# artonson/autoinst

Hardware: AMD Instinct MI355X
Metric: chunks/sec (200k-pt TARL+Spatial NCuts chunk: affinity build + recursive normalized cut) (higher is better)
Workload: dtype f64; 1 GPU; configs[1]: single 200k-point surface chunk, TARL(96-d)+Spatial affinities, alpha=1 theta=0.5 T=0.03; per GPU per step 2 batched calls of 12 chunks (one pool of iterating segments each) taken from a queue by 2 host threads; 1 builder thread(s) build the next batches' affinity graphs meanwhile; n_points=200000, nnz=7311156, threads_per_gpu=2, builder_threads_per_gpu=1, chunks_per_batch=12, parallelism=chunk-dp1

## Files before the change

autoinst_amd/csrc/ai_affinity.hip:

```cpp
#include <cstring>

#include <rocprim/device/device_radix_sort.hpp>

#include "ai_common.h"

namespace {

struct Grid {
  double minx, miny, minz, inv_cell;
  int nx, ny, nz;
};

__device__ __forceinline__ uint32_t part1by2(uint32_t x) {
  x &= 0x3ffu;
  x = (x ^ (x << 16)) & 0xff0000ffu;
  x = (x ^ (x << 8)) & 0x0300f00fu;
  x = (x ^ (x << 4)) & 0x030c30c3u;
  x = (x ^ (x << 2)) & 0x09249249u;
  return x;
}

__device__ __forceinline__ void cell_of(const Grid& g, double x, double y, double z, int& cx, int& cy, int& cz) {
  cx = (int)floor((x - g.minx) * g.inv_cell);
  cy = (int)floor((y - g.miny) * g.inv_cell);
// ... 682 lines not shown
  AI_TRY(idx.alloc(n));
  hipLaunchKernelGGL(k_cell_keys, dim3(gb), dim3(AI_BLOCK), 0, st, d_xyz, n, g, key.p, idx.p);
  AI_KERNEL_CHECK();

  ai_csr* A = new ai_csr();
  A->n = n;
  A->nnz = 0;
  A->rowptr = nullptr;
  A->col = nullptr;
  A->val = nullptr;
  A->orig = nullptr;
  A->device = ctx->device;
  ai_register_graph(ctx, A);
  auto fail = [&](int s) {
    ai_csr_free(ctx, A);
    return s;
  };
#define AI_TRYF(expr)                \
  do {                               \
    int _s = (expr);                 \
    if (_s != AI_OK) return fail(_s); \
  } while (0)
#define AI_HIPF(expr)                                                                     \
  do {                                                                                    \
    hipError_t _e = (expr);                                                               \
    if (_e != hipSuccess) {                                                               \
      ai_set_error("%s:%d: %s -> %s", __FILE__, __LINE__, #expr, hipGetErrorString(_e)); \
      return fail((_e == hipErrorOutOfMemory) ? AI_ERR_OOM : AI_ERR_HIP);                \
    }                                                                                     \
  } while (0)

  AI_HIPF(ctx->graphs.alloc((void**)&A->orig, (size_t)n * sizeof(int32_t)));
  AI_HIPF(ctx->graphs.alloc((void**)&A->rowptr, (size_t)(n + 1) * sizeof(int32_t)));
  {
    size_t tmp_bytes = 0;
    AI_HIPF(rocprim::radix_sort_pairs(nullptr, tmp_bytes, key.p, key2.p, idx.p, A->orig, (size_t)n, 0, 30, st));
    DevBuf<uint8_t> tmp;
    AI_TRYF(tmp.alloc(tmp_bytes));
    AI_HIPF(rocprim::radix_sort_pairs(tmp.p, tmp_bytes, key.p, key2.p, idx.p, A->orig, (size_t)n, 0, 30, st));
    if (!ai_current_arena()) AI_HIPF(hipStreamSynchronize(st));
  }
  AI_TRYF(X.alloc(n));
  AI_TRYF(Y.alloc(n));
  AI_TRYF(Z.alloc(n));
  AI_TRYF(cellid.alloc(n));
  AI_TRYF(cstart.alloc(ncell));
  AI_TRYF(cend.alloc(ncell));
  AI_TRYF(cnt.alloc(n + 1));
  AI_TRYF(scantmp.alloc(ai_scan_tmp_elems(n)));
  hipLaunchKernelGGL(k_gather_sorted, dim3(gb), dim3(AI_BLOCK), 0, st, d_xyz, A->orig, n, g, X.p, Y.p, Z.p, cellid.p);
  AI_HIPF(hipGetLastError());
  AI_HIPF(hipMemsetAsync(cstart.p, 0xff, (size_t)ncell * sizeof(int32_t), st));
  AI_HIPF(hipMemsetAsync(cend.p, 0, (size_t)ncell * sizeof(int32_t), st));
  hipLaunchKernelGGL(k_cell_ranges, dim3(gb), dim3(AI_BLOCK), 0, st, cellid.p, n, cstart.p, cend.p);
  AI_HIPF(hipGetLastError());
  const unsigned gnb = (unsigned)((n * AI_NB_LANES + AI_BLOCK - 1) / AI_BLOCK);
  constexpr int AI_NB_STASH = 128;
  DevBuf<int32_t> stash_col;
  DevBuf<double> stash_dist;
  AI_TRYF(stash_col.alloc((size_t)n * AI_NB_STASH));
  AI_TRYF(stash_dist.alloc((size_t)n * AI_NB_STASH));
  hipLaunchKernelGGL(k_neighbours<false>, dim3(gnb), dim3(AI_BLOCK), 0, st, X.p, Y.p, Z.p, cellid.p, cstart.p, cend.p, n, g,
                     radius, cnt.p, (const int32_t*)nullptr, (int32_t*)nullptr, (double*)nullptr, stash_col.p, stash_dist.p, AI_NB_STASH,
                     (const int32_t*)nullptr);
  AI_HIPF(hipGetLastError());
  DevBuf<unsigned long long> total;
// ... 120 lines not shown
```

autoinst_amd/csrc/ai_api.hip:

```cpp
#include <stdarg.h>
#include <string.h>

#include <algorithm>
#include <stdlib.h>
#include <hip/hip_ext.h>
#include "ai_common.h"

static thread_local char g_err[1024] = "";

void ai_set_error(const char* fmt, ...) {
  va_list ap;
  va_start(ap, fmt);
  vsnprintf(g_err, sizeof(g_err), fmt, ap);
  va_end(ap);
}

extern "C" const char* ai_last_error(void) { return g_err; }
extern "C" int ai_abi_version(void) { return AI_ABI_VERSION; }
extern "C" int64_t ai_abi_sizeof(int which) {
  return which == 0 ? (int64_t)sizeof(ai_ncut_opts) : which == 1 ? (int64_t)sizeof(ai_ncut_stats) : -1;
}

static thread_local ai_arena* g_arena = nullptr;
ai_arena* ai_current_arena() { return g_arena; }
// ... 255 lines not shown
  out[3] = (int64_t)ctx->graphs.cached_bytes;
  return AI_OK;
}

extern "C" int ai_ctx_destroy(ai_ctx* ctx) {
  if (!ctx) return AI_OK;
  ctx->helper.stop();
  (void)hipSetDevice(ctx->device);
  if (ctx->stream) (void)hipStreamSynchronize(ctx->stream);
  for (int i = 0; i < 8; ++i)
    if (ctx->ev[i]) (void)hipEventDestroy(ctx->ev[i]);
  if (ctx->side) (void)hipStreamSynchronize(ctx->side);
  for (int i = 0; i < AI_CHECK_DEPTH; ++i) {
    if (ctx->chk_ev[i]) (void)hipEventDestroy(ctx->chk_ev[i]);
    if (ctx->chk_ev1[i]) (void)hipEventDestroy(ctx->chk_ev1[i]);
  }
  if (ctx->side) (void)hipStreamDestroy(ctx->side);
  if (ctx->wave) {
    (void)hipStreamSynchronize(ctx->wave);
    (void)hipStreamDestroy(ctx->wave);
  }
  for (int i = 0; i < AI_FLOW_EVENTS; ++i)
    if (ctx->fev[i]) (void)hipEventDestroy(ctx->fev[i]);
  if (ctx->fpin) (void)hipHostFree(ctx->fpin);
  if (ctx->pinned) (void)hipHostFree(ctx->pinned);
  if (ctx->stage) (void)hipHostFree(ctx->stage);
  {
    std::lock_guard<std::mutex> lock(ctx->graphs_mu);
    for (ai_csr* g : ctx->live_graphs) {
      g->rowptr = nullptr;
      g->col = nullptr;
      g->val = nullptr;
      g->orig = nullptr;
      g->owner = nullptr;
    }
    ctx->live_graphs.clear();
  }
  ctx->arena.release_all();
  ctx->graphs.release_all();
  if (ctx->stream) (void)hipStreamDestroy(ctx->stream);
  delete ctx;
  return AI_OK;
}

extern "C" int ai_csr_free(ai_ctx* ctx, ai_csr* csr) {
  (void)ctx;
  if (!csr) return AI_OK;
  if (ai_ctx* o = csr->owner) {
    (void)hipSetDevice(o->device);
    {
      std::lock_guard<std::mutex> lock(o->graphs_mu);
      for (size_t i = 0; i < o->live_graphs.size(); ++i)
        if (o->live_graphs[i] == csr) {
          o->live_graphs.erase(o->live_graphs.begin() + i);
          break;
        }
    }
    o->graphs.release(csr->rowptr);
    o->graphs.release(csr->col);
    o->graphs.release(csr->val);
    o->graphs.release(csr->orig);
  }
  delete csr;
  return AI_OK;
}

extern "C" int ai_csr_dims(const ai_csr* csr, int64_t* n, int64_t* nnz) {
  if (!csr) {
    ai_set_error("ai_csr_dims: csr is null");
    return AI_ERR_BAD_ARG;
  }
  if (n) *n = csr->n;
  if (nnz) *nnz = csr->nnz;
  return AI_OK;
}

extern "C" int ai_csr_from_host(ai_ctx* ctx, int64_t n, const int64_t* indptr, const int32_t* indices, const double* data,
                                ai_csr** out) {
  if (!ctx || !indptr || !out || n <= 0) {
    ai_set_error("ai_csr_from_host: bad argument");
    return AI_ERR_BAD_ARG;
  }
  const int64_t nnz = indptr[n];
  if (indptr[0] != 0 || nnz < 0 || nnz >= ((int64_t)1 << 31) || n >= ((int64_t)1 << 30) || (nnz > 0 && (!indices || !data))) {
    ai_set_error("ai_csr_from_host: indptr[0] = %lld, nnz = %lld out of range", (long long)indptr[0], (long long)nnz);
    return AI_ERR_BAD_ARG;
  }
  std::vector<int32_t> rp((size_t)n + 1);
  for (int64_t i = 0; i <= n; ++i) {
    if (i > 0 && indptr[i] < indptr[i - 1]) {
      ai_set_error("ai_csr_from_host: indptr decreases at row %lld", (long long)i);
      return AI_ERR_BAD_ARG;
    }
    rp[(size_t)i] = (int32_t)indptr[i];
// ... 116 lines not shown
```

autoinst_amd/csrc/ai_common.h:

```cpp
#pragma once
#include <hip/hip_runtime.h>
#include <stdint.h>
#include <stdio.h>
#include <condition_variable>
#include <functional>
#include <mutex>
#include <atomic>
#include <thread>
#include <string>
#include <vector>

#include "../../include/autoinst_hip.h"

void ai_set_error(const char* fmt, ...);

#define AI_HIP(expr)                                                                      \
  do {                                                                                    \
    hipError_t _e = (expr);                                                               \
    if (_e != hipSuccess) {                                                               \
      ai_set_error("%s:%d: %s -> %s", __FILE__, __LINE__, #expr, hipGetErrorString(_e)); \
      return (_e == hipErrorOutOfMemory) ? AI_ERR_OOM : AI_ERR_HIP;                      \
    }                                                                                     \
  } while (0)

// ... 86 lines not shown
  hipEvent_t ev[8];
  int num_cu;
  int32_t* pinned;
  hipEvent_t chk_ev[AI_CHECK_DEPTH];
  hipEvent_t chk_ev1[AI_CHECK_DEPTH];
  hipStream_t side;
  hipStream_t wave = nullptr;
  char* fpin = nullptr;
  hipEvent_t fev[AI_FLOW_EVENTS] = {};
  ai_arena arena;
  ai_graph_cache graphs;
  char* stage;
  std::mutex graphs_mu;
  std::vector<ai_csr*> live_graphs;
  ai_helper helper;
};
void ai_register_graph(ai_ctx* ctx, ai_csr* g);
#define AI_CHECK_GRAPH(g, who)                                          \
  do {                                                                  \
    if ((g) && !(g)->rowptr) {                                          \
      ai_set_error("%s: the graph's context was destroyed", (who));     \
      return AI_ERR_BAD_ARG;                                            \
    }                                                                   \
  } while (0)

struct ai_csr {
  int64_t n;
  int64_t nnz;
  int32_t* rowptr;
  int32_t* col;
  double* val;
  int32_t* orig;
  int device;
  ai_ctx* owner = nullptr;
};

template <typename T>
struct DevBuf {
  T* p = nullptr;
  size_t count = 0;
  bool owned = false;
  DevBuf() {}
  DevBuf(const DevBuf&) = delete;
  DevBuf& operator=(const DevBuf&) = delete;
  ~DevBuf() { release(); }
  void release() {
    if (p && owned) (void)hipFree(p);
    p = nullptr;
    count = 0;
    owned = false;
  }
  int alloc(size_t n) {
    release();
    if (n == 0) n = 1;
    if (ai_arena* a = ai_current_arena()) {
      p = (T*)a->alloc(n * sizeof(T));
      if (!p) {
        ai_set_error("device workspace of %zu bytes could not be allocated", n * sizeof(T));
        return AI_ERR_OOM;
      }
      count = n;
      return AI_OK;
    }
    hipError_t e = hipMalloc((void**)&p, n * sizeof(T));
    if (e != hipSuccess) {
      p = nullptr;
// ... 114 lines not shown
```

autoinst_amd/csrc/ai_dense_sym.h:

```cpp
#pragma once
#include <algorithm>
#include <cmath>
#include <vector>

inline void cf_jacobi(std::vector<double> a, int B, std::vector<double>& evals, std::vector<double>& q) {
  q.assign((size_t)B * B, 0.0);
  for (int i = 0; i < B; ++i) q[(size_t)i * B + i] = 1.0;
  for (int sweep = 0; sweep < 60; ++sweep) {
    double off = 0.0, diag = 0.0;
    for (int i = 0; i < B; ++i) {
      diag += a[(size_t)i * B + i] * a[(size_t)i * B + i];
      for (int j = i + 1; j < B; ++j) off += a[(size_t)i * B + j] * a[(size_t)i * B + j];
    }
    if (off <= 1e-32 * std::max(diag, 1e-300)) break;
    for (int p = 0; p < B - 1; ++p)
      for (int r = p + 1; r < B; ++r) {
        const double apr = a[(size_t)p * B + r];
        if (fabs(apr) < 1e-300) continue;
        const double app = a[(size_t)p * B + p], arr = a[(size_t)r * B + r];
        const double tau = (arr - app) / (2.0 * apr);
        const double t = (tau >= 0.0 ? 1.0 : -1.0) / (fabs(tau) + sqrt(1.0 + tau * tau));
        const double c = 1.0 / sqrt(1.0 + t * t), s = t * c;
        for (int k = 0; k < B; ++k) {
          const double akp = a[(size_t)k * B + p], akr = a[(size_t)k * B + r];
          a[(size_t)k * B + p] = c * akp - s * akr;
          a[(size_t)k * B + r] = s * akp + c * akr;
        }
        for (int k = 0; k < B; ++k) {
          const double apk = a[(size_t)p * B + k], ark = a[(size_t)r * B + k];
          a[(size_t)p * B + k] = c * apk - s * ark;
          a[(size_t)r * B + k] = s * apk + c * ark;
        }
        for (int k = 0; k < B; ++k) {
          const double qkp = q[(size_t)k * B + p], qkr = q[(size_t)k * B + r];
          q[(size_t)k * B + p] = c * qkp - s * qkr;
          q[(size_t)k * B + r] = s * qkp + c * qkr;
// ... 156 lines not shown
```

autoinst_amd/csrc/ai_flow.inc:

```

struct RangeAlloc {
  std::map<int, int> fr;
  void init(int cap) {
    fr.clear();
    fr[0] = cap;
  }
  int alloc(int n) {
    for (auto it = fr.begin(); it != fr.end(); ++it)
      if (it->second >= n) {
        const int b = it->first, len = it->second;
        fr.erase(it);
        if (len > n) fr[b + n] = len - n;
        return b;
      }
    return -1;
  }
  void release(int b, int n) {
    auto it = fr.emplace(b, n).first;
    auto nx = std::next(it);
    if (nx != fr.end() && it->first + it->second == nx->first) {
      it->second += nx->second;
      fr.erase(nx);
    }
    if (it != fr.begin()) {
      auto pv = std::prev(it);
      if (pv->first + pv->second == it->first) {
        pv->second += it->second;
        fr.erase(it);
      }
    }
  }
};

struct FSeg {
  int g0 = 0, n = 0, chunk = 0, par = 0;
  int slot = -1;
  int t0 = 0, cap = 0;
  int f0 = -1, c0 = -1;
  int m = 0;
  int aux = 0;
  bool frozen = false;
  bool binary_child = false;
  int vdelta = 0;
  int warm_n = 0;
  int restarts = 0;
  double prev_true = 0.0;
};

static inline int fk_nf(int n) { return (n + AI_FINE_ROWS - 1) / AI_FINE_ROWS; }
static inline int fk_nc(int n) { return (n + AI_COARSE_ROWS - 1) / AI_COARSE_ROWS; }

class Flow {
 public:
  static constexpr int RING = 16;
  static constexpr size_t UPSLOT_BYTES = (size_t)256 << 10;
  static constexpr size_t PIN_UP = AI_FLOW_UPSLOTS * UPSLOT_BYTES;
  static constexpr size_t STATUS_BYTES = (size_t)64 << 10;
  static constexpr size_t PIN_STATUS = STATUS_BYTES;
  static constexpr size_t PIN_RES = (size_t)1 << 20;
  static constexpr size_t PIN_HIST = (size_t)16 << 20;
  static constexpr size_t PIN_COEF = (size_t)8 << 20;
  static constexpr size_t PIN_TOTAL = PIN_UP + PIN_STATUS + PIN_RES + PIN_HIST + PIN_COEF;
  static constexpr int TS_CAP = 1 << 16;
  static constexpr int AHEAD = 10;
  static constexpr int AHEAD_SMALL = 8;

  explicit Flow(ai_ctx* c) : ctx(c), sm(c->stream), ss(c->side) {}
  ai_ctx* ctx;
  hipStream_t sm, ss, sw = nullptr;
  ai_ncut_opts opt{1e-10, 4000, 16, 0, 0};
  bool clock_spmv = false;
  ai_ncut_stats stats{};
  int N = 0;
  int64_t E = 0;
  int nchunks = 0;
  const int64_t* off = nullptr;
  const int64_t* n_orig = nullptr;
  double T = 0.0;
  int SMAX = 0, WCAP = 0, FCAP = 0, CCAP = 0, FLIST = 0, CLIST = 0, mcap = 0;
  int W = 0;
  RangeAlloc sa;
  std::vector<int> chunk_sbase, chunk_live;
  std::deque<int> waiting;
  std::vector<FSeg> new_roots;
  int64_t window_rows = 0;
  FlowCsr G{};
  DevBuf<int2> rowse0, rowse1;
  DevBuf<int32_t> col1, orig1;
  DevBuf<double> w1;
  DevBuf<double> deg, sinv, sinv2, u1, wm, ev, Z;
  DevBuf<double> ev2, warmv;
  int warm = (getenv("AI_FLOW_WARM") && atoi(getenv("AI_FLOW_WARM")) == 0) ? 0 : 1;
  DevBuf<uint8_t> bin;
  DevBuf<int32_t> flag, fscan, map, newcnt, nscan, parent, rcnt, rc, ord, key, key_out, val, sorted_rows, final_order, scantmp;
  DevBuf<uint8_t> sorttmp;
  DevBuf<uint16_t> lidx;
  DevBuf<int32_t> ucol;
  DevBuf<TaskEnc> enc;
  DevBuf<int32_t> factive, cactive;
  DevBuf<double> pA;
  DevBuf<double2> pB0, pB1;
  DevBuf<int32_t> s_frozen, s_m, s_lastm, s_nextm;
  DevBuf<double> s_theta, s_resid, alpha_hist, b_hist, g_hist;
#ifdef AI_TRACE_HIST
  DevBuf<int4> sig_i, chk_i;
  DevBuf<double2> sig_d;
  DevBuf<double> chk_d;
#endif
  DevBuf<unsigned long long> work, tstamps, tblock;
  DevBuf<int32_t> dprog;
  DevBuf<int32_t> chk_ctr, chk_queue;
  DevBuf<double*> d_slabtab;
  DevBuf<FTask> d_ft[RING];
  DevBuf<CTask> d_ct[RING];
  DevBuf<PoolSeg> d_ps[RING];
  DevBuf<SegRec> d_poolrec;
  DevBuf<SegRec> wrecP, wrecC;
  DevBuf<Task> fineP, coarseP, fineC, coarseC;
  DevBuf<double> pvol, psweep, w_scale, w_thr, w_vol, coef_d;
  DevBuf<double2> presid;
  long long n_restarted = 0;
  const char* guard_log = getenv("AI_FLOW_GUARD_LOG");
  std::vector<double> hist_copy;
  std::vector<double> coef_copy;
  double max_true_resid = 0.0;
// ... 134 lines not shown
  int sync_slabtab() {
    if (slabtab_n == slabs.size()) return AI_OK;
    if (slabs.size() > 500) {
      ai_set_error("internal: more than 500 Lanczos slabs");
      return AI_ERR_INTERNAL;
    }
    double** tab = (double**)(pin_res() + PIN_RES / 2);
    for (size_t i = 0; i < slabs.size(); ++i) tab[i] = slabs[i];
    AI_HIP(hipMemcpyAsync(d_slabtab.p, tab, slabs.size() * sizeof(double*), hipMemcpyHostToDevice, sm));
    slabtab_n = slabs.size();
    return AI_OK;
  }

  static void make_recs(const std::vector<FSeg>& segs, std::vector<SegRec>& out, int& nf, int& nc) {
    out.resize(segs.size());
    nf = nc = 0;
    for (size_t i = 0; i < segs.size(); ++i) {
      const FSeg& s = segs[i];
      SegRec r;
      r.g0 = s.g0;
      r.n = s.n;
      r.slot = s.slot;
      r.par = s.par;
      r.f0 = s.f0;
      r.c0 = s.c0;
      r.foff = nf;
      r.coff = nc;
      r.t0 = s.t0;
      r.cap = s.cap;
      r.idx = (int)i;
      r.aux = s.aux;
      r.vdelta = s.vdelta;
      r.pad0 = s.warm_n;
      r.pad1 = r.pad2 = 0;
      out[i] = r;
      nf += fk_nf(s.n);
      nc += fk_nc(s.n);
    }
  }

  int setup(const ai_csr* A, int nchunks_, const int64_t* off_, const int64_t* n_orig_, double T_) {
    AI_TRY(ensure_ctx());
    N = (int)A->n;
    E = A->nnz;
    nchunks = nchunks_;
    off = off_;
    n_orig = n_orig_;
    T = T_;
    mcap = std::max(1, opt.max_iter);
    {
      int64_t big = 0;
      for (int c = 0; c < nchunks; ++c) big = std::max<int64_t>(big, off[c + 1] - off[c]);
      if (window_rows <= 0) window_rows = 4800000;
      W = (int)std::min<int64_t>(N, std::max<int64_t>(window_rows, big));
      sa.init(W);
      chunk_sbase.assign(nchunks, -1);
      chunk_live.assign(nchunks, 0);
    }
    if (opt.check_every > 64) opt.check_every = 64;
    SMAX = std::min(208 * nchunks + 64, (int)(STATUS_BYTES / sizeof(int32_t)));
#ifdef AI_TEST_HOOKS
    if (const char* e = getenv("AI_FLOW_SMAX")) SMAX = std::max(4, std::min(SMAX, atoi(e)));
#endif
    WCAP = 2 * SMAX;
    FCAP = 2 * (N / AI_FINE_ROWS + SMAX) + 64;
    CCAP = 2 * (N / AI_COARSE_ROWS + SMAX) + 64;
    FLIST = N / AI_FINE_ROWS + WCAP + 64;
    CLIST = N / AI_COARSE_ROWS + WCAP + 64;
    const size_t n = (size_t)N, e = (size_t)E;
    AI_TRY(rowse0.alloc(n));
    AI_TRY(rowse1.alloc(n));
    AI_TRY(col1.alloc(e));
    AI_TRY(w1.alloc(e));
    AI_TRY(orig1.alloc(n));
    G.rowse[0] = rowse0.p;
    G.rowse[1] = rowse1.p;
    G.col[0] = A->col;
    G.col[1] = col1.p;
    G.w[0] = A->val;
    G.w[1] = w1.p;
    G.orig[0] = A->orig;
    G.orig[1] = orig1.p;
    AI_TRY(deg.alloc(n));
    AI_TRY(sinv.alloc(n));
    AI_TRY(sinv2.alloc(n));
    AI_TRY(u1.alloc(n));
    AI_TRY(wm.alloc(e + 8));
    AI_TRY(ev.alloc(n));
    AI_TRY(Z.alloc(n));
    if (warm) {
      AI_TRY(ev2.alloc(n));
      AI_TRY(warmv.alloc(n));
    }
    AI_TRY(bin.alloc(n));
    AI_TRY(flag.alloc(n + 1));
    AI_TRY(fscan.alloc(n + 1));
    AI_TRY(map.alloc(n));
    AI_TRY(newcnt.alloc(n + 1));
    AI_TRY(nscan.alloc(n + 1));
    AI_TRY(parent.alloc(n));
    AI_TRY(rcnt.alloc(n));
    AI_TRY(rc.alloc(n + 1));
    AI_TRY(ord.alloc(n + 1));
    AI_TRY(key.alloc(n));
    AI_TRY(key_out.alloc(n));
    AI_TRY(val.alloc(n));
    AI_TRY(sorted_rows.alloc(n));
    AI_TRY(final_order.alloc(n));
    AI_TRY(scantmp.alloc(ai_scan_tmp_elems((int64_t)n)));
    AI_TRY(lidx.alloc(e + 8));
    AI_TRY(ucol.alloc(e + 8));
    AI_TRY(enc.alloc((size_t)FCAP));
    AI_TRY(factive.alloc((size_t)FCAP));
    AI_TRY(cactive.alloc((size_t)CCAP));
    AI_TRY(pA.alloc((size_t)FCAP));
    AI_TRY(pB0.alloc((size_t)CCAP));
    AI_TRY(pB1.alloc((size_t)CCAP));
    AI_TRY(s_frozen.alloc((size_t)SMAX));
    AI_TRY(s_m.alloc((size_t)SMAX));
    AI_TRY(s_lastm.alloc((size_t)SMAX));
    AI_TRY(s_nextm.alloc((size_t)SMAX));
    AI_TRY(s_theta.alloc((size_t)SMAX));
    AI_TRY(s_resid.alloc((size_t)SMAX));
    AI_TRY(alpha_hist.alloc((size_t)SMAX * mcap));
    AI_TRY(b_hist.alloc((size_t)SMAX * (mcap + 1)));
// ... 864 lines not shown
      size_t take = 0;
      for (; take < wC.size(); ++take) {
        FSeg& s = wC[take];
        if (free_slots.empty() || (int)take >= room) break;
        const int f0 = fa.alloc(fk_nf(s.n));
        const int c0 = (f0 >= 0) ? ca.alloc(fk_nc(s.n)) : -1;
        if (f0 < 0 || c0 < 0) {
          if (f0 >= 0) fa.release(f0, fk_nf(s.n));
          break;
        }
        s.aux = (int)take;
        s.slot = free_slots.back();
        free_slots.pop_back();
        ((volatile int32_t*)pin_status())[s.slot] = 0;
        s.f0 = f0;
        s.c0 = c0;
        s.cap = std::max(1, std::min(opt.max_iter, s.n - 1));
        s.frozen = false;
        s.m = 0;
      }
      if (take < wC.size()) {
        stats_deferred += (long long)(wC.size() - take);
        for (size_t i = take; i < wC.size(); ++i) {
          FSeg s = wC[i];
          s.binary_child = true;
          s.slot = -1;
          s.f0 = s.c0 = -1;
          new_roots.push_back(s);
        }
        wC.resize(take);
        w_nbin = std::min(w_nbin, (int)take);
      }
    }
    if (!wC.empty()) {
      int nfC = 0, ncC = 0;
      AI_TRY(expand(wC, wrecC, fineC.p, coarseC.p, 1, nfC, ncC));
      hipLaunchKernelGGL(fk_degree, dim3(nfC), dim3(AI_BLOCK), 0, sw, (const Task*)fineC.p, G, deg.p, sinv.p, pvol.p);
      AI_KERNEL_CHECK();
      hipLaunchKernelGGL(fk_seg_sum, dim3((unsigned)wC.size()), dim3(AI_BLOCK), 0, sw, (const SegRec*)wrecC.p, (const double*)pvol.p, w_vol.p);
      AI_KERNEL_CHECK();
      if (w_nbin > 0) {
        int nfb = 0, ncb = 0;
        for (int i = 0; i < w_nbin; ++i) {
          nfb += fk_nf(wC[i].n);
          ncb += fk_nc(wC[i].n);
        }
        hipLaunchKernelGGL(fk_cc_init, dim3(nfb), dim3(AI_BLOCK), 0, sw, (const Task*)fineC.p, G, parent.p, w_ncomp.p);
        AI_KERNEL_CHECK();
        hipLaunchKernelGGL(fk_cc_sample, dim3(nfb), dim3(AI_BLOCK), 0, sw, (const Task*)fineC.p, G, parent.p);
        AI_KERNEL_CHECK();
        hipLaunchKernelGGL(fk_cc_compress, dim3(ncb), dim3(AI_BLOCK), 0, sw, (const Task*)coarseC.p, parent.p);
        AI_KERNEL_CHECK();
        hipLaunchKernelGGL(fk_cc_hook, dim3(nfb), dim3(AI_BLOCK), 0, sw, (const Task*)fineC.p, (const SegRec*)wrecC.p, G, parent.p);
        AI_KERNEL_CHECK();
        hipLaunchKernelGGL(fk_cc_compress, dim3(ncb), dim3(AI_BLOCK), 0, sw, (const Task*)coarseC.p, parent.p);
        AI_KERNEL_CHECK();
        hipLaunchKernelGGL(fk_cc_count, dim3(ncb), dim3(AI_BLOCK), 0, sw, (const Task*)coarseC.p, (const int32_t*)parent.p, w_ncomp.p);
        AI_KERNEL_CHECK();
      }
      const FlowLz L = lz();
      const int32_t* gate = w_ncomp.p;
      hipLaunchKernelGGL(fk_scale, dim3(nfC), dim3(AI_BLOCK), 0, sw, (const Task*)fineC.p, (const SegRec*)wrecC.p, G, (const double*)deg.p,
                         (const double*)sinv.p, (const double*)w_vol.p, wm.p, sinv2.p, u1.p, gate, w_nbin);
      AI_KERNEL_CHECK();
      hipLaunchKernelGGL(fk_encode, dim3(nfC), dim3(AI_BLOCK), 0, sw, (const Task*)fineC.p, G, ucol.p, lidx.p, enc.p, gate, w_nbin);
      AI_KERNEL_CHECK();
      hipLaunchKernelGGL(fk_reset_slots, dim3(((unsigned)wC.size() + AI_BLOCK - 1) / AI_BLOCK), dim3(AI_BLOCK), 0, sw, (const SegRec*)wrecC.p,
                         (int)wC.size(), L, s_lastm.p, s_nextm.p, opt.check_every, s_theta.p, s_resid.p, gate, w_nbin, (int32_t*)(pin_res() + 64));
      AI_KERNEL_CHECK();
      hipLaunchKernelGGL(fk_lz_init, dim3(ncC), dim3(AI_BLOCK), 0, sw, (const Task*)coarseC.p, (const SegRec*)wrecC.p, G, (const double*)u1.p, slabs[0],
                         pB0.p, cactive.p, gate, w_nbin, warm ? (const double*)warmv.p : (const double*)nullptr);
      AI_KERNEL_CHECK();
      hipLaunchKernelGGL(fk_set_flags, dim3((nfC + AI_BLOCK - 1) / AI_BLOCK), dim3(AI_BLOCK), 0, sw, (const Task*)fineC.p, nfC, factive.p, gate, w_nbin);
      AI_KERNEL_CHECK();
    }
    AI_HIP(hipEventRecord(wave_ev(), sw));
    wstate = W_S3;
    return AI_OK;
  }

  int wave_finish() {
    const int32_t* r_ncomp = (const int32_t*)(pin_res() + 64);
    int joined = 0;
    for (size_t i = 0; i < wC.size(); ++i) {
      FSeg s = wC[i];
      if ((int)i < w_nbin && r_ncomp[i] != 1) {
        if (r_ncomp[i] < 1) {
          ai_set_error("internal: %d components counted in a %d-row child", r_ncomp[i], s.n);
          return AI_ERR_INTERNAL;
        }
        free_slots.push_back(s.slot);
        fa.release(s.f0, fk_nf(s.n));
        ca.release(s.c0, fk_nc(s.n));
        s.slot = -1;
        s.f0 = s.c0 = -1;
        if (T > 0.0) {
          pend_multi.push_back(s);
        } else {
          leaf(s.g0);
          --chunk_live[s.chunk];
        }
        continue;
// ... 223 lines not shown
```

autoinst_amd/csrc/ai_flow_kernels.inc:

```

struct FlowCsr {
  int2* rowse[2];
  int32_t* col[2];
  double* w[2];
  int32_t* orig[2];
};

#define FK_PAR(tk) (((tk).w >> 1) & 1)

struct __attribute__((aligned(16))) SegRec {
  int32_t g0, n;
  int32_t slot;
  int32_t par;
  int32_t f0, c0;
  int32_t foff, coff;
  int32_t t0, cap;
  int32_t idx;
  int32_t aux;
  int32_t vdelta;
  int32_t pad0, pad1, pad2;
};

#define FK_NF(sr) (((sr).n + AI_FINE_ROWS - 1) / AI_FINE_ROWS)
#define FK_NC(sr) (((sr).n + AI_COARSE_ROWS - 1) / AI_COARSE_ROWS)

__global__ __launch_bounds__(AI_BLOCK) void fk_rowse_from_rowptr(const int32_t* __restrict__ rowptr, int32_t n, int2* __restrict__ rowse) {
  const int i = blockIdx.x * AI_BLOCK + threadIdx.x;
  if (i < n) rowse[i] = make_int2(rowptr[i], rowptr[i + 1]);
}

__global__ __launch_bounds__(AI_BLOCK) void fk_degree(const Task* __restrict__ tasks, FlowCsr G, double* __restrict__ deg,
                                                      double* __restrict__ sinv, double* __restrict__ pvol) {
  __shared__ double sm[AI_BLOCK / 64];
  const Task tk = tasks[blockIdx.x];
  const int2* __restrict__ rowse = G.rowse[FK_PAR(tk)];
  const double* __restrict__ wraw = G.w[FK_PAR(tk)];
  const int l = threadIdx.x & (AI_LPR - 1), r = threadIdx.x / AI_LPR;
  double acc = 0.0;
  for (int row = tk.x + r; row < tk.y; row += AI_BLOCK / AI_LPR) {
    const int2 se = rowse[row];
    const int p0 = se.x, p1 = se.y;
    double s = 0.0;
    {
      double w[AI_ROW_PF];
#pragma unroll
      for (int q = 0; q < AI_ROW_PF; ++q) {
        const int p = p0 + l + q * AI_LPR;
        w[q] = (p < p1) ? wraw[p] : 0.0;
      }
#pragma unroll
      for (int q = 0; q < AI_ROW_PF; ++q)
        if (p0 + l + q * AI_LPR < p1) s += w[q];
    }
// ... 328 lines not shown
    ps.n = sr.n;
    ps.g0 = sr.g0;
    ps.t0 = sr.t0;
    ps.f0 = sr.f0;
    ps.f1 = sr.f0 + nf;
    ps.c0 = sr.c0;
    ps.c1 = sr.c0 + nc;
    ps.cap = sr.cap;
    ps.par = sr.par;
    ps.pad1 = ps.pad2 = 0;
    pool[blockIdx.x] = ps;
  }
}

__global__ __launch_bounds__(AI_BLOCK) void fk_reset_slots(const SegRec* __restrict__ recs, int n, FlowLz L, int32_t* __restrict__ lastm,
                                                           int32_t* __restrict__ nextm, int first_check, double* __restrict__ theta,
                                                           double* __restrict__ resid, const int32_t* __restrict__ gate, int nbin,
                                                           int32_t* __restrict__ ncomp_host) {
  const int i = blockIdx.x * AI_BLOCK + threadIdx.x;
  if (i >= n) return;
  if (i < nbin) __hip_atomic_store(&ncomp_host[i], gate[i], __ATOMIC_RELAXED, __HIP_MEMORY_SCOPE_SYSTEM);
  if (i < nbin && gate[i] != 1) return;
  const int s = recs[i].slot;
  ai_st_agent(&L.frozen[s], 0);
  ai_st_agent(&L.m[s], 0);
  ai_st_agent(&lastm[s], 0);
  ai_st_agent(&nextm[s], (int32_t)first_check);
  ai_st_agent(&theta[s], 0.0);
  ai_st_agent(&resid[s], 0.0);
}

__device__ __forceinline__ const double* fk_vec(double* const* __restrict__ slabs, size_t stride, int j) {
  return slabs[j / AI_SLAB_VECS] + (size_t)(j % AI_SLAB_VECS) * stride;
}

__global__ __launch_bounds__(AI_BLOCK) void fk_lz_init(const Task* __restrict__ ctasks, const SegRec* __restrict__ recs, FlowCsr G,
                                                       const double* __restrict__ u1, double* __restrict__ R0, double2* __restrict__ pB0,
                                                       int32_t* __restrict__ cactive, const int32_t* __restrict__ gate, int nbin,
                                                       const double* __restrict__ warm) {
  __shared__ double sm[AI_BLOCK / 64];
  const Task tk = ctasks[blockIdx.x];
  if (tk.z < nbin && gate[tk.z] != 1) return;
  R0 += recs[tk.z].vdelta;
  const int wn = warm ? recs[tk.z].pad0 : 0;
  const double wscale = sqrt((double)wn);
  const int32_t* __restrict__ orig = G.orig[FK_PAR(tk)];
  double nn = 0.0, gg = 0.0;
  for (int row = tk.x + threadIdx.x; row < tk.y; row += AI_BLOCK) {
    double r = ai_hash_unit((uint32_t)orig[row]);
    if (wn > 0) r = fma(warm[row], wscale, 1e-3 * r);
    R0[row] = r;
    nn = fma(r, r, nn);
    gg = fma(u1[row], r, gg);
  }
  const double tn = ai_block_sum(nn, sm);
  const double tg = ai_block_sum(gg, sm);
  if (threadIdx.x == 0) {
    pB0[tk.w >> 2] = make_double2(tn, tg);
    ai_st_agent(&cactive[tk.w >> 2], 1);
  }
}
__global__ __launch_bounds__(AI_BLOCK) void fk_set_flags(const Task* __restrict__ ftasks, int n, int32_t* __restrict__ factive,
                                                         const int32_t* __restrict__ gate, int nbin) {
  const int i = blockIdx.x * AI_BLOCK + threadIdx.x;
  if (i >= n) return;
  const Task t = ftasks[i];
// ... 1252 lines not shown
```

autoinst_amd/csrc/ai_ncut.hip:

```cpp
#include <math.h>
#include <stdlib.h>
#include <string.h>

#include <algorithm>
#include <deque>
#include <map>

#include <rocprim/device/device_radix_sort.hpp>

#include "ai_common.h"

#include "ai_ncut_params.h"
#include "ai_ncut_shared.h"
#include "ai_tridiag.h"

namespace {
#include "ai_flow_kernels.inc"
#include "ai_flow.inc"
__global__ __launch_bounds__(AI_BLOCK) void k_offset_copy(int32_t* __restrict__ dst, const int32_t* __restrict__ src, int64_t n,
                                                          int32_t add) {
  const int64_t i = (int64_t)blockIdx.x * AI_BLOCK + threadIdx.x;
  if (i < n) dst[i] = (src ? src[i] : (int32_t)i) + add;
}
}

#ifdef AI_WITH_LOCKSTEP
__attribute__((visibility("hidden"))) int ncut_lockstep(ai_ctx* ctx, const ai_csr* csr, int nchunks, const int64_t* off, const int64_t* n_orig, double T,
                                                        double split_lim, const ai_ncut_opts* opts, int32_t* const* labels_out, int32_t* n_groups,
                                                        ai_ncut_stats* stats_out, double t0);
#endif

static int ncut_impl(ai_ctx* ctx, const ai_csr* csr, int nchunks, const int64_t* off, const int64_t* n_orig, double T, double split_lim,
                     const ai_ncut_opts* opts, int32_t* const* labels_out, int32_t* n_groups, ai_ncut_stats* stats_out, double t0) {
  static const int lockstep = getenv("AI_NCUT_LOCKSTEP") ? atoi(getenv("AI_NCUT_LOCKSTEP")) : 0;
#ifdef AI_WITH_LOCKSTEP
  if (lockstep) return ncut_lockstep(ctx, csr, nchunks, off, n_orig, T, split_lim, opts, labels_out, n_groups, stats_out, t0);
#else
  if (lockstep) {
    ai_set_error("AI_NCUT_LOCKSTEP=1: this build has no level-synchronous driver (load libautoinst_hip_lockstep.so: make -C autoinst_amd/csrc lockstep)");
    return AI_ERR_BAD_ARG;
  }
#endif
  return ncut_flow(ctx, csr, nchunks, off, n_orig, T, split_lim, opts, labels_out, n_groups, stats_out, t0);
}
// ... 19 lines not shown
  }
  int64_t N = 0, E = 0;
  for (int c = 0; c < count; ++c) {
    if (!graphs[c] || !labels_out[c] || num_points_orig[c] < 0) {
      ai_set_error("ai_ncut_batch: null graph / label buffer at position %d", c);
      return AI_ERR_BAD_ARG;
    }
    AI_CHECK_GRAPH(graphs[c], "ai_ncut_batch");
    N += graphs[c]->n;
    E += graphs[c]->nnz;
  }
  if (N >= ((int64_t)1 << 30) || E >= ((int64_t)1 << 31)) {
    ai_set_error("ai_ncut_batch: %lld rows / %lld entries exceed the int32 index range of this build", (long long)N, (long long)E);
    return AI_ERR_BAD_ARG;
  }
  AI_HIP(hipSetDevice(ctx->device));
  const double t0 = now_ms();
  ArenaScope arena_scope(&ctx->arena);
  hipStream_t st = ctx->stream;
  std::vector<int> order;
  for (int pass = 0; pass < 2; ++pass)
    for (int c = 0; c < count; ++c)
      if (eligible((int)graphs[c]->n, num_points_orig[c], split_lim) == (pass == 0)) order.push_back(c);
  std::vector<int64_t> norig_p(count);
  std::vector<int32_t*> labels_p(count);
  std::vector<int32_t> ngroups_p(count, 0);
  DevBuf<int32_t> rp, cl, og;
  DevBuf<double> vl;
  AI_TRY(rp.alloc((size_t)N + 1));
  AI_TRY(cl.alloc((size_t)E));
  AI_TRY(vl.alloc((size_t)E));
  AI_TRY(og.alloc((size_t)N));
  std::vector<int64_t> off(count + 1, 0);
  int64_t eoff = 0;
  for (int c = 0; c < count; ++c) {
    const ai_csr* g = graphs[order[c]];
    norig_p[c] = num_points_orig[order[c]];
    labels_p[c] = labels_out[order[c]];
    const int64_t n = g->n, e = g->nnz;
    off[c + 1] = off[c] + n;
    hipLaunchKernelGGL(k_offset_copy, dim3((unsigned)((n + 1 + AI_BLOCK - 1) / AI_BLOCK)), dim3(AI_BLOCK), 0, st, rp.p + off[c],
                       (const int32_t*)g->rowptr, n + 1, (int32_t)eoff);
    AI_KERNEL_CHECK();
    if (e) {
      hipLaunchKernelGGL(k_offset_copy, dim3((unsigned)((e + AI_BLOCK - 1) / AI_BLOCK)), dim3(AI_BLOCK), 0, st, cl.p + eoff, (const int32_t*)g->col,
                         e, (int32_t)off[c]);
      AI_KERNEL_CHECK();
      AI_HIP(hipMemcpyAsync(vl.p + eoff, g->val, (size_t)e * sizeof(double), hipMemcpyDeviceToDevice, st));
    }
    hipLaunchKernelGGL(k_offset_copy, dim3((unsigned)((n + AI_BLOCK - 1) / AI_BLOCK)), dim3(AI_BLOCK), 0, st, og.p + off[c],
                       (const int32_t*)g->orig, n, 0);
    AI_KERNEL_CHECK();
    eoff += e;
  }
  ai_csr merged;
  merged.n = N;
  merged.nnz = E;
  merged.rowptr = rp.p;
  merged.col = cl.p;
  merged.val = vl.p;
  merged.orig = og.p;
  merged.device = ctx->device;
  const int rc = ncut_impl(ctx, &merged, count, off.data(), norig_p.data(), T, split_lim, opts, labels_p.data(), ngroups_p.data(), stats_out, t0);
  for (int c = 0; c < count; ++c) n_groups[order[c]] = ngroups_p[c];
  return rc;
}
```

Before: 140.7 chunks/sec.

## Warm-start Lanczos with PCA principal-axis projection of segment coordinates

The affinity graph now keeps a copy of the point coordinates, and the batched ncut passes per-chunk coordinate pointers into the flow solver. For segments with no existing warm vector, three new kernels compute the 3D coordinate moments, take the principal axis with a 3x3 Jacobi solve, and fill the warm-start vector with each point's projection onto that axis. The aim is to start the eigensolver closer to the Fiedler vector so fewer Lanczos iterations and restarts are needed. The cost is an extra device copy of xyz per graph, more graph memory, and three extra kernel launches per wave of new segments.

```diff
diff --git a/autoinst_amd/csrc/ai_affinity.hip b/autoinst_amd/csrc/ai_affinity.hip
--- a/autoinst_amd/csrc/ai_affinity.hip
+++ b/autoinst_amd/csrc/ai_affinity.hip
@@ -738,6 +738,8 @@
 
   AI_HIPF(ctx->graphs.alloc((void**)&A->orig, (size_t)n * sizeof(int32_t)));
   AI_HIPF(ctx->graphs.alloc((void**)&A->rowptr, (size_t)(n + 1) * sizeof(int32_t)));
+  AI_HIPF(ctx->graphs.alloc((void**)&A->xyz, (size_t)n * 3 * sizeof(double)));
+  AI_HIPF(hipMemcpyAsync(A->xyz, d_xyz, (size_t)n * 3 * sizeof(double), hipMemcpyDeviceToDevice, st));
   {
     size_t tmp_bytes = 0;
     AI_HIPF(rocprim::radix_sort_pairs(nullptr, tmp_bytes, key.p, key2.p, idx.p, A->orig, (size_t)n, 0, 30, st));
diff --git a/autoinst_amd/csrc/ai_api.hip b/autoinst_amd/csrc/ai_api.hip
--- a/autoinst_amd/csrc/ai_api.hip
+++ b/autoinst_amd/csrc/ai_api.hip
@@ -311,6 +311,7 @@
       g->col = nullptr;
       g->val = nullptr;
       g->orig = nullptr;
+      g->xyz = nullptr;
       g->owner = nullptr;
     }
     ctx->live_graphs.clear();
@@ -339,6 +340,7 @@
     o->graphs.release(csr->col);
     o->graphs.release(csr->val);
     o->graphs.release(csr->orig);
+    o->graphs.release(csr->xyz);
   }
   delete csr;
   return AI_OK;
diff --git a/autoinst_amd/csrc/ai_common.h b/autoinst_amd/csrc/ai_common.h
--- a/autoinst_amd/csrc/ai_common.h
+++ b/autoinst_amd/csrc/ai_common.h
@@ -142,6 +142,8 @@
   double* val;
   int32_t* orig;
   int device;
+  double* xyz = nullptr;
+  const double* const* chunk_xyz = nullptr;
   ai_ctx* owner = nullptr;
 };
 
diff --git a/autoinst_amd/csrc/ai_dense_sym.h b/autoinst_amd/csrc/ai_dense_sym.h
--- a/autoinst_amd/csrc/ai_dense_sym.h
+++ b/autoinst_amd/csrc/ai_dense_sym.h
@@ -2,6 +2,54 @@
 #include <algorithm>
 #include <cmath>
 #include <vector>
+
+#ifdef __HIPCC__
+#define AI_DENSE_HD __host__ __device__
+#else
+#define AI_DENSE_HD
+#endif
+
+AI_DENSE_HD inline double ai_jacobi3(const double a6[6], double e[3]) {
+  double a[3][3] = {{a6[0], a6[1], a6[2]}, {a6[1], a6[3], a6[4]}, {a6[2], a6[4], a6[5]}};
+  double q[3][3] = {{1.0, 0.0, 0.0}, {0.0, 1.0, 0.0}, {0.0, 0.0, 1.0}};
+  for (int sweep = 0; sweep < 60; ++sweep) {
+    const double off = a[0][1] * a[0][1] + a[0][2] * a[0][2] + a[1][2] * a[1][2];
+    const double diag = a[0][0] * a[0][0] + a[1][1] * a[1][1] + a[2][2] * a[2][2];
+    if (!(off > 1e-32 * fmax(diag, 1e-300))) break;
+    for (int p = 0; p < 2; ++p)
+      for (int r = p + 1; r < 3; ++r) {
+        const double apr = a[p][r];
+        if (fabs(apr) < 1e-300) continue;
+        const double tau = (a[r][r] - a[p][p]) / (2.0 * apr);
+        const double t = (tau >= 0.0 ? 1.0 : -1.0) / (fabs(tau) + sqrt(1.0 + tau * tau));
+        const double c = 1.0 / sqrt(1.0 + t * t), s = t * c;
+        for (int k = 0; k < 3; ++k) {
+          const double akp = a[k][p], akr = a[k][r];
+          a[k][p] = c * akp - s * akr;
+          a[k][r] = s * akp + c * akr;
+        }
+        for (int k = 0; k < 3; ++k) {
+          const double apk = a[p][k], ark = a[r][k];
+          a[p][k] = c * apk - s * ark;
+          a[r][k] = s * apk + c * ark;
+        }
+        for (int k = 0; k < 3; ++k) {
+          const double qkp = q[k][p], qkr = q[k][r];
+          q[k][p] = c * qkp - s * qkr;
+          q[k][r] = s * qkp + c * qkr;
+        }
+      }
+  }
+  int j = 0;
+  if (a[1][1] > a[j][j]) j = 1;
+  if (a[2][2] > a[j][j]) j = 2;
+  int big = 0;
+  if (fabs(q[1][j]) > fabs(q[big][j])) big = 1;
+  if (fabs(q[2][j]) > fabs(q[big][j])) big = 2;
+  const double sg = q[big][j] < 0.0 ? -1.0 : 1.0;
+  for (int k = 0; k < 3; ++k) e[k] = sg * q[k][j];
+  return a[j][j];
+}
 
 inline void cf_jacobi(std::vector<double> a, int B, std::vector<double>& evals, std::vector<double>& q) {
   q.assign((size_t)B * B, 0.0);
diff --git a/autoinst_amd/csrc/ai_flow.inc b/autoinst_amd/csrc/ai_flow.inc
--- a/autoinst_amd/csrc/ai_flow.inc
+++ b/autoinst_amd/csrc/ai_flow.inc
@@ -43,6 +43,7 @@
   bool binary_child = false;
   int vdelta = 0;
   int warm_n = 0;
+  int pca = 0;
   int restarts = 0;
   double prev_true = 0.0;
 };
@@ -91,6 +92,10 @@
   DevBuf<double> deg, sinv, sinv2, u1, wm, ev, Z;
   DevBuf<double> ev2, warmv;
   int warm = (getenv("AI_FLOW_WARM") && atoi(getenv("AI_FLOW_WARM")) == 0) ? 0 : 1;
+  std::vector<const double*> h_xyz;
+  bool any_xyz = false;
+  DevBuf<const double*> d_xyz;
+  DevBuf<double> pca_part, pca_axis;
   DevBuf<uint8_t> bin;
   DevBuf<int32_t> flag, fscan, map, newcnt, nscan, parent, rcnt, rc, ord, key, key_out, val, sorted_rows, final_order, scantmp;
   DevBuf<uint8_t> sorttmp;
@@ -291,7 +296,8 @@
       r.aux = s.aux;
       r.vdelta = s.vdelta;
       r.pad0 = s.warm_n;
-      r.pad1 = r.pad2 = 0;
+      r.pad1 = s.pca;
+      r.pad2 = 0;
       out[i] = r;
       nf += fk_nf(s.n);
       nc += fk_nc(s.n);
@@ -350,6 +356,17 @@
     if (warm) {
       AI_TRY(ev2.alloc(n));
       AI_TRY(warmv.alloc(n));
+      h_xyz.assign((size_t)nchunks, nullptr);
+      for (int c = 0; c < nchunks; ++c) {
+        h_xyz[c] = A->chunk_xyz ? A->chunk_xyz[c] : (nchunks == 1 ? (const double*)A->xyz : nullptr);
+        any_xyz |= h_xyz[c] != nullptr;
+      }
+      if (any_xyz) {
+        AI_TRY(d_xyz.alloc((size_t)nchunks));
+        AI_TRY(pca_part.alloc((size_t)FK_PCA_VALS * CCAP));
+        AI_TRY(pca_axis.alloc((size_t)8 * WCAP));
+        AI_HIP(hipMemcpyAsync(d_xyz.p, h_xyz.data(), (size_t)nchunks * sizeof(const double*), hipMemcpyHostToDevice, sm));
+      }
     }
     AI_TRY(bin.alloc(n));
     AI_TRY(flag.alloc(n + 1));
@@ -1280,6 +1297,11 @@
         w_nbin = std::min(w_nbin, (int)take);
       }
     }
+    bool any_pca = false;
+    for (FSeg& s : wC) {
+      s.pca = (any_xyz && s.warm_n == 0 && h_xyz[s.chunk]) ? s.chunk + 1 : 0;
+      any_pca |= s.pca != 0;
+    }
     if (!wC.empty()) {
       int nfC = 0, ncC = 0;
       AI_TRY(expand(wC, wrecC, fineC.p, coarseC.p, 1, nfC, ncC));
@@ -1316,6 +1338,17 @@
       hipLaunchKernelGGL(fk_reset_slots, dim3(((unsigned)wC.size() + AI_BLOCK - 1) / AI_BLOCK), dim3(AI_BLOCK), 0, sw, (const SegRec*)wrecC.p,
                          (int)wC.size(), L, s_lastm.p, s_nextm.p, opt.check_every, s_theta.p, s_resid.p, gate, w_nbin, (int32_t*)(pin_res() + 64));
       AI_KERNEL_CHECK();
+      if (any_pca) {
+        hipLaunchKernelGGL(fk_pca_moments, dim3(ncC), dim3(AI_BLOCK), 0, sw, (const Task*)coarseC.p, (const SegRec*)wrecC.p, G,
+                           (const double* const*)d_xyz.p, pca_part.p, (size_t)CCAP, gate, w_nbin);
+        AI_KERNEL_CHECK();
+        hipLaunchKernelGGL(fk_pca_axis, dim3((unsigned)wC.size()), dim3(AI_BLOCK), 0, sw, wrecC.p, G, (const double* const*)d_xyz.p,
+                           (const double*)pca_part.p, (size_t)CCAP, pca_axis.p, gate, w_nbin);
+        AI_KERNEL_CHECK();
+        hipLaunchKernelGGL(fk_pca_fill, dim3(ncC), dim3(AI_BLOCK), 0, sw, (const Task*)coarseC.p, (const SegRec*)wrecC.p, G,
+                           (const double* const*)d_xyz.p, (const double*)pca_axis.p, (const double*)u1.p, warmv.p, gate, w_nbin);
+        AI_KERNEL_CHECK();
+      }
       hipLaunchKernelGGL(fk_lz_init, dim3(ncC), dim3(AI_BLOCK), 0, sw, (const Task*)coarseC.p, (const SegRec*)wrecC.p, G, (const double*)u1.p, slabs[0],
                          pB0.p, cactive.p, gate, w_nbin, warm ? (const double*)warmv.p : (const double*)nullptr);
       AI_KERNEL_CHECK();
diff --git a/autoinst_amd/csrc/ai_flow_kernels.inc b/autoinst_amd/csrc/ai_flow_kernels.inc
--- a/autoinst_amd/csrc/ai_flow_kernels.inc
+++ b/autoinst_amd/csrc/ai_flow_kernels.inc
@@ -18,7 +18,9 @@
   int32_t idx;
   int32_t aux;
   int32_t vdelta;
-  int32_t pad0, pad1, pad2;
+  int32_t pad0;
+  int32_t pad1;
+  int32_t pad2;
 };
 
 #define FK_NF(sr) (((sr).n + AI_FINE_ROWS - 1) / AI_FINE_ROWS)
@@ -413,6 +415,93 @@
 
 __device__ __forceinline__ const double* fk_vec(double* const* __restrict__ slabs, size_t stride, int j) {
   return slabs[j / AI_SLAB_VECS] + (size_t)(j % AI_SLAB_VECS) * stride;
+}
+
+#define FK_PCA_VALS 9
+__global__ __launch_bounds__(AI_BLOCK) void fk_pca_moments(const Task* __restrict__ ctasks, const SegRec* __restrict__ recs, FlowCsr G,
+                                                           const double* const* __restrict__ xyz_tab, double* __restrict__ part, size_t pstride,
+                                                           const int32_t* __restrict__ gate, int nbin) {
+  __shared__ double sm[AI_BLOCK / 64];
+  const Task tk = ctasks[blockIdx.x];
+  if (tk.z < nbin && gate[tk.z] != 1) return;
+  const SegRec sr = recs[tk.z];
+  if (sr.pad1 == 0) return;
+  const double* __restrict__ xyz = xyz_tab[sr.pad1 - 1];
+  const int32_t* __restrict__ orig = G.orig[FK_PAR(tk)];
+  const size_t o0 = (size_t)3 * (size_t)orig[sr.g0];
+  const double rx = xyz[o0], ry = xyz[o0 + 1], rz = xyz[o0 + 2];
+  double s[FK_PCA_VALS] = {0.0, 0.0, 0.0, 0.0, 0.0, 0.0, 0.0, 0.0, 0.0};
+  for (int row = tk.x + threadIdx.x; row < tk.y; row += AI_BLOCK) {
+    const size_t o = (size_t)3 * (size_t)orig[row];
+    const double dx = xyz[o] - rx, dy = xyz[o + 1] - ry, dz = xyz[o + 2] - rz;
+    s[0] += dx;
+    s[1] += dy;
+    s[2] += dz;
+    s[3] = fma(dx, dx, s[3]);
+    s[4] = fma(dx, dy, s[4]);
+    s[5] = fma(dx, dz, s[5]);
+    s[6] = fma(dy, dy, s[6]);
+    s[7] = fma(dy, dz, s[7]);
+    s[8] = fma(dz, dz, s[8]);
+  }
+#pragma unroll
+  for (int k = 0; k < FK_PCA_VALS; ++k) {
+    const double tot = ai_block_sum(s[k], sm);
+    if (threadIdx.x == 0) part[(size_t)k * pstride + (size_t)(tk.w >> 2)] = tot;
+  }
+}
+
+__global__ __launch_bounds__(AI_BLOCK) void fk_pca_axis(SegRec* __restrict__ recs, FlowCsr G, const double* const* __restrict__ xyz_tab,
+                                                        const double* __restrict__ part, size_t pstride, double* __restrict__ axis,
+                                                        const int32_t* __restrict__ gate, int nbin) {
+  __shared__ double sm[AI_BLOCK / 64];
+  const int i = blockIdx.x;
+  if (i < nbin && gate[i] != 1) return;
+  const SegRec sr = recs[i];
+  if (sr.pad1 == 0) return;
+  double s[FK_PCA_VALS];
+#pragma unroll
+  for (int k = 0; k < FK_PCA_VALS; ++k) s[k] = ai_range_sum(part + (size_t)k * pstride, sr.c0, sr.c0 + FK_NC(sr), sm);
+  if (threadIdx.x != 0) return;
+  const double inv = 1.0 / (double)sr.n;
+  const double mx = s[0] * inv, my = s[1] * inv, mz = s[2] * inv;
+  const double cov[6] = {s[3] * inv - mx * mx, s[4] * inv - mx * my, s[5] * inv - mx * mz,
+                         s[6] * inv - my * my, s[7] * inv - my * mz, s[8] * inv - mz * mz};
+  double e[3];
+  const double sigma = sqrt(ai_jacobi3(cov, e));
+  const double* __restrict__ xyz = xyz_tab[sr.pad1 - 1];
+  const size_t o0 = (size_t)3 * (size_t)G.orig[sr.par][sr.g0];
+  const double cx = xyz[o0] + mx, cy = xyz[o0 + 1] + my, cz = xyz[o0 + 2] + mz;
+  if (!(sigma > 0.0) || !(fabs(sigma) + fabs(cx) + fabs(cy) + fabs(cz) <= 1.7976931348623157e308)) return;
+  double* a = axis + (size_t)8 * i;
+  a[0] = e[0];
+  a[1] = e[1];
+  a[2] = e[2];
+  a[3] = cx;
+  a[4] = cy;
+  a[5] = cz;
+  a[6] = sqrt((double)sr.n) / sigma;
+  a[7] = sigma;
+  recs[i].pad0 = sr.n;
+}
+
+__global__ __launch_bounds__(AI_BLOCK) void fk_pca_fill(const Task* __restrict__ ctasks, const SegRec* __restrict__ recs, FlowCsr G,
+                                                        const double* const* __restrict__ xyz_tab, const double* __restrict__ axis,
+                                                        const double* __restrict__ u1, double* __restrict__ warm,
+                                                        const int32_t* __restrict__ gate, int nbin) {
+  const Task tk = ctasks[blockIdx.x];
+  if (tk.z < nbin && gate[tk.z] != 1) return;
+  const SegRec sr = recs[tk.z];
+  if (sr.pad1 == 0 || sr.pad0 == 0) return;
+  const double* __restrict__ xyz = xyz_tab[sr.pad1 - 1];
+  const int32_t* __restrict__ orig = G.orig[FK_PAR(tk)];
+  const double* __restrict__ a = axis + (size_t)8 * tk.z;
+  const double ex = a[0], ey = a[1], ez = a[2], cx = a[3], cy = a[4], cz = a[5], sc = a[6];
+  for (int row = tk.x + threadIdx.x; row < tk.y; row += AI_BLOCK) {
+    const size_t o = (size_t)3 * (size_t)orig[row];
+    const double t = fma(xyz[o + 2] - cz, ez, fma(xyz[o + 1] - cy, ey, (xyz[o] - cx) * ex));
+    warm[row] = (u1[row] * t) * sc;
+  }
 }
 
 __global__ __launch_bounds__(AI_BLOCK) void fk_lz_init(const Task* __restrict__ ctasks, const SegRec* __restrict__ recs, FlowCsr G,
diff --git a/autoinst_amd/csrc/ai_ncut.hip b/autoinst_amd/csrc/ai_ncut.hip
--- a/autoinst_amd/csrc/ai_ncut.hip
+++ b/autoinst_amd/csrc/ai_ncut.hip
@@ -10,6 +10,7 @@
 
 #include "ai_common.h"
 
+#include "ai_dense_sym.h"
 #include "ai_ncut_params.h"
 #include "ai_ncut_shared.h"
 #include "ai_tridiag.h"
@@ -95,9 +96,11 @@
   AI_TRY(vl.alloc((size_t)E));
   AI_TRY(og.alloc((size_t)N));
   std::vector<int64_t> off(count + 1, 0);
+  std::vector<const double*> chunk_xyz(count);
   int64_t eoff = 0;
   for (int c = 0; c < count; ++c) {
     const ai_csr* g = graphs[order[c]];
+    chunk_xyz[c] = g->xyz;
     norig_p[c] = num_points_orig[order[c]];
     labels_p[c] = labels_out[order[c]];
     const int64_t n = g->n, e = g->nnz;
@@ -124,6 +127,7 @@
   merged.val = vl.p;
   merged.orig = og.p;
   merged.device = ctx->device;
+  merged.chunk_xyz = chunk_xyz.data();
   const int rc = ncut_impl(ctx, &merged, count, off.data(), norig_p.data(), T, split_lim, opts, labels_p.data(), ngroups_p.data(), stats_out, t0);
   for (int c = 0; c < count; ++c) n_groups[order[c]] = ngroups_p[c];
   return rc;
```

Result: faster. 147.3 chunks/sec (median of 6 runs) (+4.7%).
